# BlockstreamResearch/secp256k1-zkp

Measured on AMD Instinct MI355X. Metric: 64-bit Borromean rangeproof verifies/sec, higher is better.
Workload: dtype u32 limbs (9x29-bit), 32x32->64 integer MAC

## Files before the change

__graft_entry__.py:

```python
import os
import subprocess
import sys

ROOT = os.path.dirname(os.path.abspath(__file__))
CSRC = os.path.join(ROOT, "secp256k1_zkp_amd", "csrc")
HIPCC = os.environ.get("HIPCC", "/opt/rocm/bin/hipcc")
HIP_FLAGS = ["--offload-arch=gfx950", "-O3", "-std=c++17", "-shared", "-fPIC", "-Wno-unused-value"]


def _run(cmd, cwd=None):
    print("+", " ".join(cmd), flush=True)
    subprocess.check_call(cmd, cwd=cwd)


def _stale(target, sources):
    if not os.path.exists(target):
        return True
    t = os.path.getmtime(target)
    return any(os.path.getmtime(s) > t for s in sources if os.path.exists(s))


def build(force=False):
    hdrs = [os.path.join(CSRC, f) for f in os.listdir(CSRC) if f.endswith((".h", ".hip"))] + [os.path.join(ROOT, "include", "secp256k1_zkp_amd.h")]
    sys.path.insert(0, ROOT)
    from secp256k1_zkp_amd import build_lib
    build_lib.build(force=force)
    prims_src = os.path.join(ROOT, "tests", "gpu_prims", "prims.hip")
    prims = os.path.join(ROOT, "tests", "gpu_prims", "libs2k_gpuprims.so")
    if force or _stale(prims, hdrs + [prims_src]):
        _run([HIPCC] + HIP_FLAGS + ["-o", prims, prims_src])
    winv_src = os.path.join(ROOT, "tests", "wave_inverse", "waveinv_test.hip")
    winv = os.path.join(ROOT, "tests", "wave_inverse", "libs2k_waveinv_test.so")
    if force or _stale(winv, hdrs + [winv_src]):
        _run([HIPCC] + HIP_FLAGS + ["-o", winv, winv_src])
    emu_src = os.path.join(ROOT, "tests", "host_emul", "hostemu.cpp")
    emu = os.path.join(ROOT, "tests", "host_emul", "libs2k_hostemu.so")
    if force or _stale(emu, hdrs + [emu_src]):
        _run(["g++", "-O2", "-std=c++17", "-fPIC", "-shared", "-o", emu, emu_src])
    ecdsa_emu_src = os.path.join(ROOT, "tests", "host_emul", "ecdsa_emu.cpp")
    ecdsa_emu = os.path.join(ROOT, "tests", "host_emul", "libs2k_ecdsa_emu.so")
    if force or _stale(ecdsa_emu, hdrs + [emu_src, ecdsa_emu_src]):
        _run(["g++", "-O2", "-std=c++17", "-fPIC", "-shared", "-o", ecdsa_emu, ecdsa_emu_src])
    if os.path.exists(os.path.join(ROOT, "oracle", "zkp_oracle.c")):
        _run(["make", "-s", "-C", os.path.join(ROOT, "oracle"), "oracle"])
    if os.path.isdir(os.environ.get("S2K_REFERENCE", "/root/reference")):
        _run(["make", "-s", "-C", os.path.join(ROOT, "oracle"), "ref", "hooked", "benches", "routed"])
    sys.path.insert(0, ROOT)
    import secp256k1_zkp_amd
    from secp256k1_zkp_amd import _native
    _native.load()


def smoke():
    sys.path.insert(0, ROOT)
    from tests import smoke_impl
    smoke_impl.run()


if __name__ == "__main__":
    build(force="--force" in sys.argv)
    if "--smoke" in sys.argv:
        smoke()
```

secp256k1_zkp_amd/csrc/engine_rangeproof.hip:

```cpp
#include "engine_internal.h"

__global__ void __launch_bounds__(256)
k_rp_header(rp_ws ws, uint64_t* min_value, uint64_t* max_value, const unsigned char* proofs, const uint64_t* proof_off, const unsigned char* gens64,
            rp_gen_dev gc, size_t n) {
    const size_t p = (size_t)blockIdx.x * blockDim.x + threadIdx.x;
    if (p >= n) return;
    if (p == 0) { ws.plan[0] = 0; ws.plan[1] = 0; ws.plan[2] = 0; ws.plan[3] = 0; }
    uint64_t mn, mx;
    rp_header(ws.rec[p], &mn, &mx, proofs + proof_off[p], proof_off[p + 1] - proof_off[p]);
    min_value[p] = mn; max_value[p] = mx;
    ws.rec[p].gslot = rp_gen_lookup(gc, gens64 + 64 * p);
}
__global__ void __launch_bounds__(192)
k_rp_prologue(rp_ws ws, const uint64_t* min_value, const unsigned char* commits33, const unsigned char* proofs,
              const uint64_t* proof_off, const unsigned char* extra, const uint64_t* extra_off, const unsigned char* gens64, size_t n) {
    __builtin_amdgcn_s_setprio(3);
    const u32 role = threadIdx.x >> 6;
    const size_t p = (size_t)blockIdx.x * 64 + (threadIdx.x & 63);
    int commit_ok = 0;
    if (p < n) {
        rp_rec& rec = ws.rec[p];
        if (role == 0) commit_ok = rp_pp_commit(rec, min_value[p], commits33 + 33 * p, gens64 + 64 * p);
        else if (role == 1) {
            const unsigned char* ex = nullptr; uint64_t exlen = 0;
            if (extra && extra_off) { ex = extra + extra_off[p]; exlen = extra_off[p + 1] - extra_off[p]; if (exlen == 0) ex = nullptr; }
            rp_pp_hash(rec, commits33 + 33 * p, proofs + proof_off[p], ex, exlen, gens64 + 64 * p);
        } else rp_pp_bases(rec, ws.bases + p * RP_MAX_RINGS * RP_GEJ_WORDS, gens64 + 64 * p, ws.dbases + p * RP_MAX_RINGS * RP_GEJ_WORDS);
    }
    __syncthreads();
    if (p < n && role == 0 && (ws.rec[p].hdr & 1u) && commit_ok) ws.rec[p].ok = 1;
}
__global__ void __launch_bounds__(256)
k_rp_lift(rp_ws ws, const unsigned char* proofs, const uint64_t* proof_off, size_t n) {
    const size_t t = (size_t)blockIdx.x * blockDim.x + threadIdx.x;
    const size_t p = t >> 5; const u32 ring = (u32)(t & 31);
    if (p >= n) return;
    const rp_rec& rec = ws.rec[p];
    if (!(rec.hdr & 1u) || ring + 1 >= rec.rings) return;
    rp_lift(rec, ws.pub0 + (p * RP_MAX_RINGS + ring) * RP_GEJ_WORDS, ws.lift_ok + p * RP_MAX_RINGS + ring, proofs + proof_off[p], ring);
}
__global__ void __launch_bounds__(64)
k_rp_sum(rp_ws ws, u32 gen_valid, size_t n) {
    const size_t p = (size_t)blockIdx.x * blockDim.x + threadIdx.x;
    u32 cF = 0, cG = 0, rings = 0;
    if (p < n) {
        rp_sum(ws.rec[p], ws.pub0 + p * RP_MAX_RINGS * RP_GEJ_WORDS, ws.lift_ok + p * RP_MAX_RINGS);
        const rp_rec& rec = ws.rec[p];
        if (rec.ok) {
            rings = rec.rings;
            const int fast = gen_valid && rec.gslot < RP_GEN_SLOTS && ((gen_valid >> rec.gslot) & 1u);
            if (fast) cF = (rings + S2K_RP_K - 1) / S2K_RP_K; else cG = rings;
        }
    }
    u32 pf = cF, pg = cG;
    for (int d = 1; d < 64; d <<= 1) {
        const u32 a = __shfl_up(pf, d), b = __shfl_up(pg, d);
        if ((int)threadIdx.x >= d) { pf += a; pg += b; }
    }
    u32 baseF = 0, baseG = 0;
    if (threadIdx.x == 63) { baseF = pf ? atomicAdd(&ws.plan[0], pf) : 0u; baseG = pg ? atomicAdd(&ws.plan[1], pg) : 0u; }
    baseF = __shfl(baseF, 63); baseG = __shfl(baseG, 63);
    u32 oF = baseF + pf - cF, oG = baseG + pg - cG;
    for (u32 g = 0; g < cF; g++) ws.mapF[oF + g] = (u32)p | (g << 20);
    for (u32 r = 0; r < cG; r++) ws.mapG[oG + r] = (u32)p | (r << 20);
}
#ifndef S2K_RINGS_WAVES
#define S2K_RINGS_WAVES 2
#endif
__global__ void __launch_bounds__(256, S2K_RINGS_WAVES)
k_rp_rings_shared(rp_ws ws, const unsigned char* __restrict__ proofs, const uint64_t* __restrict__ proof_off, const u32* __restrict__ gtab, u32* __restrict__ ptab, u32* ev,
                  rp_gen_dev gc, u32 dbg) {
    const size_t t = (size_t)blockIdx.x * blockDim.x + threadIdx.x;
    const u32 nF = ws.plan[0];
    if ((t & ~size_t(63)) >= nF) return;
    const int live = t < nF;
    const u32 item = ws.mapF[live ? t : 0];
    const size_t p = item & 0xFFFFFu; const u32 g = item >> 20;
    const rp_rec& rec = ws.rec[p];
    __shared__ u32 s_dig[S2K_RING_DIG_WORDS * 256];
    const u32 sl = rec.gslot < RP_GEN_SLOTS ? rec.gslot : gc.any;
    const size_t lanes = (size_t)gridDim.x * 256, wave = t >> 6, lane = t & 63;
    u32* const raw0 = ptab + lanes * S2K_RP_K * S2K_RTAB_WORDS;
    const rp_shared_mem M{ptab + t * S2K_RP_K * S2K_RTAB_WORDS, raw0 + wave * S2K_RRAW_WAVE_WORDS + lane,
                          raw0 + (lanes >> 6) * S2K_RRAW_WAVE_WORDS + wave * (S2K_RP_K * RP_PARK_WORDS * 64) + lane, S2K_LANE_DIG(s_dig)};
    const int served = rp_rings_shared<S2K_RP_K>(rec, ws.pub0 + (p * RP_MAX_RINGS + g * S2K_RP_K) * RP_GEJ_WORDS, ws.ring_out + p * RP_RING_OUT_BYTES, ws.ring_ok + p * RP_MAX_RINGS,
                                                 proofs + proof_off[p], g * S2K_RP_K, live, gtab, gc.tab[sl], gc.xmul[sl], M, ev ? ev + p * (RP_MAX_RINGS * 32) : nullptr, dbg);
    if (served != RP_SHARED_SERVED && live) {
        const u32 r0 = g * S2K_RP_K, cnt = rec.rings - r0 < S2K_RP_K ? rec.rings - r0 : S2K_RP_K;
        const u32 base = atomicAdd(&ws.plan[1], cnt);
        for (u32 i = 0; i < cnt; i++) ws.mapG[base + i] = (u32)p | ((r0 + i) << 20);
        atomicAdd(&ws.plan[served == RP_SHARED_SUSPECT ? 2 : 3], cnt);
    }
}
__global__ void __launch_bounds__(256, S2K_RINGS_WAVES)
k_rp_rings(rp_ws ws, const unsigned char* __restrict__ proofs, const uint64_t* __restrict__ proof_off, const u32* __restrict__ gtab, u32* __restrict__ ptab, u32* ev, int split) {
    const size_t t = (size_t)blockIdx.x * blockDim.x + threadIdx.x;
    const u32 nG = ws.plan[1];
    if ((t & ~size_t(63)) >= nG) return;
    const int live = t < nG;
    const u32 item = ws.mapG[live ? t : 0];
    const size_t p = item & 0xFFFFFu; const u32 ring = item >> 20;
    const rp_rec& rec = ws.rec[p];
    __shared__ u32 s_dig[S2K_DIG_WORDS * 256];
    const lane_mem lm{ptab + t * S2K_PTAB_WORDS, S2K_LANE_DIG(s_dig)};
    rp_ring(rec, ws.bases + (p * RP_MAX_RINGS + ring) * RP_GEJ_WORDS, ws.pub0 + (p * RP_MAX_RINGS + ring) * RP_GEJ_WORDS,
            ws.ring_out + p * RP_RING_OUT_BYTES + ring * 33, ws.ring_ok + p * RP_MAX_RINGS + ring, proofs + proof_off[p], ring, live, gtab, lm, ev ? ev + (p * RP_MAX_RINGS + ring) * 32 : nullptr,
            split ? ws.dbases + (p * RP_MAX_RINGS + ring) * RP_GEJ_WORDS : (const u32*)nullptr, split ? ws.tcur + (p * RP_MAX_RINGS + ring) * RP_GEJ_WORDS : (u32*)nullptr);
}
__global__ void __launch_bounds__(64)
k_rp_final(rp_ws ws, int32_t* results, const unsigned char* proofs, const uint64_t* proof_off, const unsigned char* gens64, rp_gen_mbox* mbox, size_t n) {
    const size_t p = (size_t)blockIdx.x * blockDim.x + threadIdx.x;
    int ok = 0; u32 gslot = RP_GSLOT_NONE;
    if (p < n) {
        ok = rp_final(ws.rec[p], ws.ring_out + p * RP_RING_OUT_BYTES, ws.ring_ok + p * RP_MAX_RINGS, proofs + proof_off[p]);
        results[p] = ok;
        gslot = ws.rec[p].gslot;
    }
    if (mbox) {
        for (u32 sl = 0; sl < RP_GEN_SLOTS; sl++) {
            const unsigned long long m = __ballot(ok && gslot == sl);
            if (m && threadIdx.x == 0) atomicAdd(&mbox->hits[sl], (u32)__popcll(m));
        }
        rp_gen_report_miss(mbox, gens64 + 64 * (p < n ? p : 0), ok && gslot == RP_GSLOT_NONE);
    }
}

struct rp_rewind_args {
    u32* ev; u32* prep; u32* secs;
    unsigned char* blind_out; uint64_t* value_out; unsigned char* msg_out; uint64_t* outlen; size_t msg_stride; const unsigned char* nonces;
};
__global__ void __launch_bounds__(64)
k_rp_rewind_draws(rp_ws ws, rp_rewind_args ra, const unsigned char* proofs, const uint64_t* proof_off, const unsigned char* gens64, size_t n) {
    const size_t p = (size_t)blockIdx.x * blockDim.x + threadIdx.x;
    if (p >= n || !ws.rec[p].ok) return;
    rp_rewind_draws(ws.rec[p], proofs + proof_off[p], ra.nonces + 32 * p, gens64 + 64 * p, ra.prep + p * 1024, ra.secs + p * 256);
}
__global__ void __launch_bounds__(256, 2)
k_rp_rewind(rp_ws ws, rp_rewind_args ra, int32_t* results, const uint64_t* min_value, const unsigned char* proofs, const uint64_t* proof_off,
            const unsigned char* gens64, const u32* gtab, u32* ptab, size_t n) {
    const size_t t = (size_t)blockIdx.x * blockDim.x + threadIdx.x;
    const int inrange = t < n;
    const size_t p = inrange ? t : 0;
    int ok = inrange && results[p];
    scalar blind; u64 value = 0, mlen = 0; sc_set_zero(blind);
    const unsigned char* proof = proofs + proof_off[p];
    if (ok) {
        mlen = (ra.msg_out && ra.outlen) ? ra.outlen[p] : 0;
        if (mlen > ra.msg_stride) mlen = ra.msg_stride;
        ok = rp_rewind_recover(blind, value, ra.msg_out ? ra.msg_out + p * ra.msg_stride : nullptr, &mlen, ws.rec[p], proof,
                               ra.ev + p * 1024, ra.prep + p * 1024, ra.secs + p * 256);
    }
    u64 vv = 0;
    if (ok) {
        u32 off; int exp, mant; u64 scale, mn, mx;
        rp_getheader(off, exp, mant, scale, &mn, &mx, proof, proof_off[p + 1] - proof_off[p]);
        vv = value * scale + min_value[p];
    }
    gej A; scalar sv;
    { ge g; fe_set_b32_mod(g.x, gens64 + 64 * p); fe_set_b32_mod(g.y, gens64 + 64 * p + 32); fe_norm_weak(g.x); fe_norm_weak(g.y); gej_set_ge(A, g); }
    sc_set_u64(sv, vv);
    if (!ok) { sc_set_zero(sv); sc_set_zero(blind); }
    __shared__ u32 s_dig[S2K_DIG_WORDS * 256];
    const lane_mem lm{ptab + t * S2K_PTAB_WORDS, S2K_LANE_DIG(s_dig)};
    gej R; ecmult_lane(R, A, sv, blind, 1, gtab, lm);
    ge a; ge_set_gej(a, R);
    if (ok) {
        fe cx, cy, d;
        for (int i = 0; i < 9; i++) { cx.n[i] = ws.rec[p].commit[i]; cy.n[i] = ws.rec[p].commit[9 + i]; }
        ok &= !R.inf;
        fe_neg(d, a.x, 1); fe_add(d, cx); ok &= fe_normalizes_to_zero(d);
        fe_neg(d, a.y, 1); fe_add(d, cy); ok &= fe_normalizes_to_zero(d);
    }
    if (inrange) {
        results[p] = ok;
        if (!ok) { sc_set_zero(blind); vv = 0; mlen = 0; }
        sc_get_b32(ra.blind_out + 32 * p, blind);
        ra.value_out[p] = vv;
        if (ra.outlen) ra.outlen[p] = mlen;
    }
}

static size_t rp_ws_bytes(size_t n) {
    return ws_need({64, (n * RP_MAX_RINGS / S2K_RP_K + 64) * 4, (n * RP_MAX_RINGS + 64) * 4, n * sizeof(rp_rec), n * RP_MAX_RINGS * RP_GEJ_WORDS * 4, n * RP_MAX_RINGS * RP_GEJ_WORDS * 4, n * RP_MAX_RINGS * RP_GEJ_WORDS * 4,
                    n * RP_MAX_RINGS * RP_GEJ_WORDS * 4, n * RP_MAX_RINGS, n * RP_RING_OUT_BYTES, n * RP_MAX_RINGS});
}
static void rp_ws_carve(rp_ws& w, ws_carver& c, size_t n) {
    w.plan = c.take<u32>(16); w.mapF = c.take<u32>(n * RP_MAX_RINGS / S2K_RP_K + 64); w.mapG = c.take<u32>(n * RP_MAX_RINGS + 64);
    w.rec = c.take<rp_rec>(n);
    w.bases = c.take<u32>(n * RP_MAX_RINGS * RP_GEJ_WORDS);
    w.pub0 = c.take<u32>(n * RP_MAX_RINGS * RP_GEJ_WORDS);
    w.dbases = c.take<u32>(n * RP_MAX_RINGS * RP_GEJ_WORDS);
    w.tcur = c.take<u32>(n * RP_MAX_RINGS * RP_GEJ_WORDS);
    w.lift_ok = c.take<unsigned char>(n * RP_MAX_RINGS);
    w.ring_out = c.take<unsigned char>(n * RP_RING_OUT_BYTES);
    w.ring_ok = c.take<unsigned char>(n * RP_MAX_RINGS);
}
int engine_rp_slots(s2k_engine* e, size_t nw) {
    const size_t bytes = (rp_ws_bytes(nw) + (size_t(1) << 20)) & ~((size_t(1) << 20) - 1);
    if (bytes <= e->rp_mem_bytes) return 1;
// ... 504 lines not shown
```

secp256k1_zkp_amd/csrc/group.h:

```cpp
#pragma once
#include "fe.h"

struct ge  { fe x, y; };
struct gej { fe x, y, z; int inf; };

#define GEJ_ADD_NEEDS_DOUBLE 1

S2K_HD void fe_set_beta(fe& r) {
    const u32 b[9] = {0x119501EEu, 0x09CB6143u, 0x1D626570u, 0x0092EA25u, 0x034E99CFu, 0x03CF561Au, 0x1C41B991u, 0x056CAF80u, 0x007AE96Au};
#pragma unroll
    for (int i = 0; i < 9; i++) r.n[i] = b[i];
}

S2K_HD void gej_set_infinity(gej& r) { fe_set_zero(r.x); fe_set_zero(r.y); fe_set_zero(r.z); r.inf = 1; }
S2K_HD void gej_set_ge(gej& r, const ge& a) { r.x = a.x; r.y = a.y; fe_set_int(r.z, 1); r.inf = 0; }
S2K_HD void ge_neg(ge& r, const ge& a) { r.x = a.x; fe_neg(r.y, a.y, 1); fe_norm_weak(r.y); }

S2K_HD void gej_double(gej& r, const gej& a) {
    fe x = a.x, y = a.y, l, s, t;
    fe_norm_weak(x); fe_norm_weak(y);
    fe_mul_sqr(r.z, y, a.z, s, y);
    fe_mul_sqr(t, x, s, l, x);
    fe_neg(t, t, 1);
    fe_mul_int(l, 3); fe_half(l);
    fe_norm_weak(l);
    fe_sqr2(r.x, l, s, s);
    fe_add(r.x, t); fe_add(r.x, t);
    fe_add(t, r.x);
    fe_mul(r.y, t, l);
    fe_add(r.y, s);
    fe_neg(r.y, r.y, 2);
    r.inf = a.inf;
}

S2K_HD int gej_add_ge(gej& r, const gej& a, const ge& b, fe* zr = nullptr) {
    fe z12, u2, s2, h, i, h2, h3, t, i2;
    fe_sqr(z12, a.z);
    fe_mul2(u2, b.x, z12, s2, b.y, z12);
    fe_neg(h, a.x, 5); fe_add(h, u2);
    fe_norm_seq(h);
    fe zz; fe_mul2(s2, s2, a.z, zz, a.z, h);
    fe_neg(i, a.y, 3); fe_add(i, s2);
    fe_norm_seq(i);
    const int hz = fe_seq_is_zero(h), iz = fe_seq_is_zero(i);
    fe_sqr2(i2, i, h2, h);
    fe_mul2(h3, h, h2, t, a.x, h2);
    if (zr) *zr = h;
    fe x3, y3, tn;
    fe_neg(x3, h3, 1);
    fe_neg(tn, t, 1);
    fe_add(x3, tn); fe_add(x3, tn); fe_add(x3, i2);
    fe_norm_weak(x3);
    fe_neg(tn, x3, 1); fe_add(tn, t);
    fe_mul2(y3, tn, i, h3, h3, a.y);
    fe_neg(h3, h3, 1);
    fe_add(y3, h3);
    const int dbl = (!a.inf) & hz & iz;
    const int inf = (!a.inf) & hz & (!iz);
    const int take_b = a.inf | dbl;
    fe one; fe_set_int(one, 1);
    fe_select(r.x, b.x, x3, take_b);
    fe_select(r.y, b.y, y3, take_b);
    fe_select(r.z, one, zz, take_b);
    r.inf = inf;
    return dbl ? GEJ_ADD_NEEDS_DOUBLE : 0;
}

S2K_HD void gej_double_lean(gej& r, const gej& a) {
    fe l, s, t, nx, w;
    fe_mul_sqr(r.z, a.y, a.z, s, a.y);
    fe_neg(nx, a.x, 1);
    fe_mul_sqr(t, nx, s, l, a.x);
    fe_mul_int(l, 3); fe_half(l);
    fe_norm_weak(l);
    fe_sqr(r.x, l);
    fe_add(r.x, t); fe_add(r.x, t);
    fe_norm_weak(r.x);
    fe_add2(w, r.x, t);
    fe_muladd<false, true>(r.y, l, w, s, s);
    fe_neg(r.y, r.y, 1);
    r.inf = 0;
}
S2K_HD int gej_add_ge_lean(gej& r, const gej& a, const ge& b) {
    fe z12, u2, s2, h, i, h2, h3, t, i2, ny, w;
    fe_sqr(z12, a.z);
    fe_mul2(u2, b.x, z12, s2, b.y, z12);
    fe_neg(h, a.x, 1); fe_add(h, u2);
    fe_norm_seq(h);
    fe_mul2(s2, s2, a.z, r.z, a.z, h);
    fe_neg(ny, a.y, 2);
    fe_add2(i, s2, ny);
    fe_norm_weak(i);
    const int hz = fe_seq_is_zero(h);
    fe_sqr2(i2, i, h2, h);
    fe_mul2(h3, h, h2, t, a.x, h2);
    fe_add2(w, t, t); fe_add(w, h3);
    fe_neg(w, w, 3);
    fe_add2(r.x, i2, w);
    fe_norm_weak(r.x);
    fe_neg(w, r.x, 1); fe_add(w, t);
    fe_muladd<false, false>(r.y, i, w, ny, h3);
    r.inf = 0;
    return hz;
}

S2K_HD void gej_add_var(gej& r, const gej& a, const gej& b) {
    fe z22, z12, u1, u2, s1, s2, h, i, h2, h3, t, i2;
    fe_sqr2(z22, b.z, z12, a.z);
    fe_mul2(u1, a.x, z22, u2, b.x, z12);
    fe_mul2(s1, a.y, z22, s2, b.y, z12);
    fe_mul2(s1, s1, b.z, s2, s2, a.z);
    fe_neg(h, u1, 1); fe_add(h, u2);
    fe_neg(i, s1, 1); fe_add(i, s2);
    fe_norm_seq(h); fe_norm_seq(i);
    const int hz = fe_seq_is_zero(h), iz = fe_seq_is_zero(i);
    gej res;
    if ((!a.inf) & (!b.inf) & hz & iz) {
        gej_double(res, a);
    } else {
        fe zz;
        fe_mul_sqr(zz, a.z, b.z, h2, h);
        fe_mul_sqr(res.z, zz, h, i2, i);
        fe_mul2(h3, h, h2, t, u1, h2);
        fe x3, tn;
        fe_neg(x3, h3, 1); fe_neg(tn, t, 1);
        fe_add(x3, tn); fe_add(x3, tn); fe_add(x3, i2);
        fe_norm_weak(x3);
        fe_neg(tn, x3, 1); fe_add(tn, t);
        fe_mul2(res.y, tn, i, h3, h3, s1);
        fe_neg(h3, h3, 1);
        fe_add(res.y, h3);
        res.x = x3;
        res.inf = hz & (!iz);
        if (a.inf) res = b;
        else if (b.inf) res = a;
    }
    r = res;
}

S2K_HD void ge_set_gej(ge& r, const gej& a) {
    fe zi, zi2, zi3;
    fe_inv(zi, a.z);
    fe_sqr(zi2, zi); fe_mul(zi3, zi2, zi);
    fe_mul(r.x, a.x, zi2); fe_mul(r.y, a.y, zi3);
    fe_normalize(r.x); fe_normalize(r.y);
}

S2K_HD void ge_curve_rhs(fe& c, const fe& x) {
    fe x2; fe_sqr(x2, x); fe_mul(c, x2, x);
    c.n[0] += 7u;
}
S2K_HD int ge_set_xquad(ge& r, const fe& x) {
    fe c; ge_curve_rhs(c, x);
    fe_norm_weak(c);
    r.x = x;
    return fe_sqrt(r.y, c);
}
S2K_HD int ge_set_xo(ge& r, const fe& x, int odd) {
    if (!ge_set_xquad(r, x)) return 0;
    fe_normalize(r.y);
    if (fe_is_odd(r.y) != odd) { fe_neg(r.y, r.y, 1); fe_normalize(r.y); }
    return 1;
}
S2K_HD int ge_is_valid(const ge& a) {
    fe y2, c; fe_sqr(y2, a.y); ge_curve_rhs(c, a.x); fe_norm_weak(c);
    return fe_equal(y2, c);
}

struct gez { fe x, y, zz, zzz; int inf; };
S2K_HD void gez_add_ge(gez& a, const ge& b) {
    if (a.inf) { a.x = b.x; a.y = b.y; fe_set_int(a.zz, 1); fe_set_int(a.zzz, 1); a.inf = 0; return; }
    fe u2, s2, p, r;
    fe_mul2(u2, b.x, a.zz, s2, b.y, a.zzz);
    fe_neg(p, a.x, 1); fe_add(p, u2);
    fe_neg(r, a.y, 3); fe_add(r, s2);
    fe_norm_seq(p); fe_norm_seq(r);
    if (fe_seq_is_zero(p)) {
        if (!fe_seq_is_zero(r)) { a.inf = 1; return; }
        gej t, d; gej_set_ge(t, b); gej_double(d, t);
        a.x = d.x; a.y = d.y; fe_norm_weak(a.x); fe_norm_weak(a.y);
        fe_sqr(a.zz, d.z); fe_mul(a.zzz, a.zz, d.z);
        return;
    }
    fe pp, rr, ppp, q;
    fe_sqr2(pp, p, rr, r);
    fe_mul2(ppp, p, pp, q, a.x, pp);
    fe x3, t1, nq, y3a, y3b;
    fe_neg(x3, ppp, 1); fe_neg(nq, q, 1);
    fe_add(x3, nq); fe_add(x3, nq); fe_add(x3, rr);
    fe_norm_weak(x3);
    fe_neg(t1, x3, 1); fe_add(t1, q);
    fe_mul2(y3a, r, t1, y3b, a.y, ppp);
    fe_mul2(a.zz, a.zz, pp, a.zzz, a.zzz, ppp);
    fe_neg(y3b, y3b, 1); fe_add(y3a, y3b);
    a.x = x3; a.y = y3a;
}
S2K_HD void gej_set_gez(gej& r, const gez& a) {
    r.inf = a.inf;
    if (a.inf) { fe_set_zero(r.x); fe_set_zero(r.y); fe_set_zero(r.z); return; }
    fe_mul2(r.x, a.x, a.zz, r.y, a.y, a.zzz);
    r.z = a.zz;
}
S2K_HD void gez_add_ge_lean(gez& a, const ge& b) {
    fe u2, s2, p, r;
    fe_mul2(u2, b.x, a.zz, s2, b.y, a.zzz);
    fe_neg(p, a.x, 1); fe_add(p, u2); fe_norm_weak(p);
    fe_neg(r, a.y, 1); fe_add(r, s2); fe_norm_weak(r);
    fe pp, rr, ppp, q;
    fe_sqr2(pp, p, rr, r);
    fe_mul2(ppp, p, pp, q, a.x, pp);
    fe x3, nq, t1, ny;
    fe_neg(x3, ppp, 1); fe_neg(nq, q, 1);
    fe_add(x3, nq); fe_add(x3, nq); fe_add(x3, rr);
    fe_norm_weak(x3);
    fe_neg(t1, x3, 1); fe_add(t1, q);
    fe_neg(ny, a.y, 1);
    fe_muladd<false, false>(a.y, r, t1, ny, ppp);
    fe_mul2(a.zz, a.zz, pp, a.zzz, a.zzz, ppp);
    a.x = x3;
}
```

secp256k1_zkp_amd/csrc/modinv.h:

```cpp
#pragma once
#include "s2k_common.h"

#define DS_LIMBS 9
#define DS_BITS 30
#define DS_MASK ((int32_t)0x3FFFFFFF)
#define DS_BATCHES 20

struct ds_int { int32_t w[DS_LIMBS]; };
struct ds_modulus { int32_t w[DS_LIMBS]; u32 inv; };

#define DS_MOD_P ds_modulus{{-977, -4, 0, 0, 0, 0, 0, 0, 65536}, 0x2DDACACFu}
#define DS_MOD_N ds_modulus{{0x10364141, 0x3F497A33, 0x348A03BB, 0x2BB739AB, 0x3FFFFEBA, 0x3FFFFFFF, 0x3FFFFFFF, 0x3FFFFFFF, 0xFFFF}, 0x2A774EC1u}

#if defined(__HIP_DEVICE_COMPILE__)
#define DS_WAVE_ANY(p) (__any(p))
#define DS_WAVE_ALL(p) (__all(p))
#define DS_UNIFORM(x) (__builtin_amdgcn_readfirstlane(x))
#else
#define DS_WAVE_ANY(p) (p)
#define DS_WAVE_ALL(p) (p)
#define DS_UNIFORM(x) (x)
#endif

S2K_HD int ds_ctz32(u32 x) { return __builtin_ctz(x | 0x80000000u); }

S2K_HD int32_t ds_batch(int32_t zeta, u32 f, u32 g, int32_t t[4]) {
    int32_t u = 1, v = 0, q = 0, r = 1;
    int left = DS_BITS;
    while (DS_WAVE_ANY(left > 0)) {
        int z = ds_ctz32(g); z = z < left ? z : left;
        g >>= z; u = (int32_t)((u32)u << z); v = (int32_t)((u32)v << z); zeta -= z; left -= z;
        const int act = left > 0;
        const int sw = act & (zeta < 0);
        const u32 fm = sw ? 0u - f : f;
        const int32_t um = sw ? -u : u, vm = sw ? -v : v;
        const u32 g2 = (g + fm) >> 1;
        const int32_t q2 = q + um, r2 = r + vm;
        f = sw ? g : f; u = sw ? q : u; v = sw ? r : v;
        g = act ? g2 : g; q = act ? q2 : q; r = act ? r2 : r;
        zeta = sw ? -zeta - 2 : zeta - act;
        u = (int32_t)((u32)u << act); v = (int32_t)((u32)v << act); left -= act;
    }
    t[0] = u; t[1] = v; t[2] = q; t[3] = r;
    return zeta;
}

S2K_HD int32_t ds_batch_uniform(int32_t zeta, u32 f, u32 g, int32_t t[4]) {
    int32_t u = 1, v = 0, q = 0, r = 1;
    int left = DS_BITS;
    for (;;) {
        int z = ds_ctz32(g); z = z < left ? z : left;
        g >>= z; u = (int32_t)((u32)u << z); v = (int32_t)((u32)v << z); zeta -= z; left -= z;
        if (left <= 0) break;
        if (zeta < 0) {
            const u32 f0 = f; const int32_t u0 = u, v0 = v;
            f = g; u = q; v = r;
            g = (g - f0) >> 1; q -= u0; r -= v0;
            zeta = -zeta - 2;
        } else {
            g = (g + f) >> 1; q += u; r += v;
            zeta -= 1;
        }
        u = (int32_t)((u32)u << 1); v = (int32_t)((u32)v << 1); left -= 1;
    }
    t[0] = u; t[1] = v; t[2] = q; t[3] = r;
    return zeta;
}

template <bool WITH_M>
S2K_HD void ds_apply(ds_int& a, ds_int& b, const int32_t t[4], const ds_modulus md) {
    const int64_t t00 = t[0], t01 = t[1], t10 = t[2], t11 = t[3];
    int64_t ca = t00 * a.w[0] + t01 * b.w[0], cb = t10 * a.w[0] + t11 * b.w[0];
    int64_t ka = 0, kb = 0;
    if (WITH_M) {
        ka = (int64_t)((0u - (u32)ca * md.inv) & (u32)DS_MASK);
        kb = (int64_t)((0u - (u32)cb * md.inv) & (u32)DS_MASK);
        ca += ka * md.w[0]; cb += kb * md.w[0];
    }
    ca >>= DS_BITS; cb >>= DS_BITS;
#pragma unroll
    for (int i = 1; i < DS_LIMBS; i++) {
        ca += t00 * a.w[i] + t01 * b.w[i];
        cb += t10 * a.w[i] + t11 * b.w[i];
        if (WITH_M && md.w[i] != 0) { ca += ka * md.w[i]; cb += kb * md.w[i]; }
        a.w[i - 1] = (int32_t)ca & DS_MASK; ca >>= DS_BITS;
        b.w[i - 1] = (int32_t)cb & DS_MASK; cb >>= DS_BITS;
    }
    a.w[DS_LIMBS - 1] = (int32_t)ca; b.w[DS_LIMBS - 1] = (int32_t)cb;
}

S2K_HD void ds_add_multiple(ds_int& r, int32_t c, const ds_modulus md) {
    int64_t acc = 0;
#pragma unroll
    for (int i = 0; i < DS_LIMBS - 1; i++) { acc += (int64_t)r.w[i] + (int64_t)c * md.w[i]; r.w[i] = (int32_t)acc & DS_MASK; acc >>= DS_BITS; }
    r.w[DS_LIMBS - 1] = (int32_t)(acc + r.w[DS_LIMBS - 1] + (int64_t)c * md.w[DS_LIMBS - 1]);
}

template <bool UNIFORM = false>
S2K_HD void ds_inverse_words(u32 o[8], const u32 w[8], const ds_modulus md) {
    ds_int f, g, d, e;
#pragma unroll
    for (int i = 0; i < DS_LIMBS; i++) {
        const int bit = DS_BITS * i, idx = bit >> 5, sh = bit & 31;
        u64 v = w[idx];
        if (idx + 1 < 8) v |= (u64)w[idx + 1] << 32;
        g.w[i] = (int32_t)((u32)(v >> sh) & (u32)DS_MASK);
        f.w[i] = md.w[i]; d.w[i] = 0; e.w[i] = 0;
    }
    e.w[0] = 1;
    int32_t zeta = -1;
#pragma unroll 1
    for (int it = 0; it < DS_BATCHES; it++) {
        int32_t t[4];
        if (UNIFORM) zeta = ds_batch_uniform(DS_UNIFORM(zeta), (u32)DS_UNIFORM(f.w[0]), (u32)DS_UNIFORM(g.w[0]), t);
        else zeta = ds_batch(zeta, (u32)f.w[0], (u32)g.w[0], t);
        ds_apply<true>(d, e, t, md);
        ds_apply<false>(f, g, t, md);
        if (it >= DS_BATCHES - 5) {
            int32_t gz = 0;
#pragma unroll
            for (int i = 0; i < DS_LIMBS; i++) gz |= g.w[i];
            if (DS_WAVE_ALL(gz == 0)) break;
        }
    }
    ds_add_multiple(d, 32, md);
    const int32_t qest = d.w[DS_LIMBS - 1] >> 16;
    ds_add_multiple(d, -qest, md);
    { ds_int s = d; ds_add_multiple(s, -1, md); const int keep = s.w[DS_LIMBS - 1] >= 0;
#pragma unroll
      for (int i = 0; i < DS_LIMBS; i++) d.w[i] = keep ? s.w[i] : d.w[i]; }
    { const int fneg = f.w[DS_LIMBS - 1] < 0;
      int32_t nz = 0;
#pragma unroll
      for (int i = 0; i < DS_LIMBS; i++) nz |= d.w[i];
      ds_int s;
#pragma unroll
      for (int i = 0; i < DS_LIMBS; i++) s.w[i] = -d.w[i];
      int64_t acc = 0;
#pragma unroll
      for (int i = 0; i < DS_LIMBS - 1; i++) { acc += (int64_t)s.w[i] + md.w[i]; s.w[i] = (int32_t)acc & DS_MASK; acc >>= DS_BITS; }
      s.w[DS_LIMBS - 1] = (int32_t)(acc + s.w[DS_LIMBS - 1] + md.w[DS_LIMBS - 1]);
      const int take = fneg & (nz != 0);
#pragma unroll
      for (int i = 0; i < DS_LIMBS; i++) d.w[i] = take ? s.w[i] : d.w[i]; }
#pragma unroll
    for (int j = 0; j < 8; j++) {
        const int bit = 32 * j, i = bit / DS_BITS, sh = bit % DS_BITS;
        u64 v = (u64)(u32)d.w[i] >> sh;
        if (i + 1 < DS_LIMBS) v |= (u64)(u32)d.w[i + 1] << (DS_BITS - sh);
        if (i + 2 < DS_LIMBS) v |= (u64)(u32)d.w[i + 2] << (2 * DS_BITS - sh);
        o[j] = (u32)v;
    }
}
```

secp256k1_zkp_amd/csrc/rangeproof.h:

```cpp
#pragma once
#include "gtable.h"
#include "sha256.h"
#include "waveinv.h"

#define RP_MAX_RINGS 32
#define RP_GEJ_WORDS 28
#define RP_RING_OUT_BYTES (RP_MAX_RINGS * 33 + 32)
#define RP_GSLOT_NONE 0xFFFFFFFFu

struct rp_rec {
    u32 ok;
    u32 rings;
    u32 last_rsize;
    u32 off_signs;
    u32 off_pts;
    u32 off_e0;
    u32 off_s;
    u32 hdr;
    u32 gslot;
    u32 m[8];
    u32 commit[18];
    u32 accj[RP_GEJ_WORDS];
};

// ... 33 lines not shown
        if (exp > 18) return 0;
        mantissa = proof[offset] + 1;
        if (mantissa > 64) return 0;
        *max_value = 0xFFFFFFFFFFFFFFFFull >> (64 - mantissa);
    } else {
        *max_value = 0;
    }
    offset += 1;
    scale = 1;
    for (int i = 0; i < exp; i++) {
        if (*max_value > 0xFFFFFFFFFFFFFFFFull / 10) return 0;
        *max_value *= 10; scale *= 10;
    }
    *min_value = 0;
    if (has_min) {
        if (plen - offset < 8) return 0;
        u64 v = 0;
        for (int i = 0; i < 8; i++) v = (v << 8) | proof[offset + i];
        *min_value = v;
        offset += 8;
    }
    if (*max_value > 0xFFFFFFFFFFFFFFFFull - *min_value) return 0;
    *max_value += *min_value;
    return 1;
}

S2K_HD void rp_header(rp_rec& rec, u64* min_value, u64* max_value, const unsigned char* proof, u64 plen) {
    rec.ok = 0; rec.rings = 0; rec.last_rsize = 0; rec.hdr = 0; rec.gslot = RP_GSLOT_NONE;
    rec.off_signs = 0; rec.off_pts = 0; rec.off_e0 = 0; rec.off_s = 0;
    *min_value = 0; *max_value = 0;
    u32 offset; int exp, mantissa; u64 scale;
    if (!rp_getheader(offset, exp, mantissa, scale, min_value, max_value, proof, plen)) return;
    u32 rings = 1, npub = 1, last_rsize = 1;
    if (mantissa != 0) {
        rings = (u32)mantissa >> 1; npub = rings * 4; last_rsize = 4;
        if (mantissa & 1) { npub += 2; rings++; last_rsize = 2; }
    }
    if (plen - offset < (u64)32 * (npub + rings - 1) + 32 + ((rings + 6) >> 3)) return;
    rec.rings = rings; rec.last_rsize = last_rsize;
    rec.off_signs = offset;
    offset += (rings + 6) >> 3;
    if ((rings - 1) & 7) {
        if ((proof[offset - 1] >> ((rings - 1) & 7)) != 0) return;
    }
    rec.off_pts = offset;
    rec.off_e0 = offset + 32 * (rings - 1);
    rec.off_s = rec.off_e0 + 32;
    if ((u64)rec.off_s + (u64)32 * npub != plen) return;
    rec.hdr = 1u | ((u32)(exp + 1) << 8);
}
S2K_HD void rp_load_generator(ge& g, const unsigned char* gen64) {
    fe_set_b32_mod(g.x, gen64); fe_set_b32_mod(g.y, gen64 + 32);
    fe_normalize(g.x); fe_normalize(g.y);
}
S2K_HD int rp_pp_commit(rp_rec& rec, u64 min_value, const unsigned char* commit33, const unsigned char* gen64) {
    if (!(rec.hdr & 1u)) return 0;
    ge c;
    int valid = (commit33[0] & 0xFEu) == 8u;
    {
        fe x; valid &= fe_set_b32_limit(x, commit33 + 1);
        valid &= ge_set_xquad(c, x);
        fe_normalize(c.x); fe_normalize(c.y);
        if (commit33[0] & 1) { fe_neg(c.y, c.y, 1); fe_normalize(c.y); }
    }
    for (int i = 0; i < 9; i++) { rec.commit[i] = c.x.n[i]; rec.commit[9 + i] = c.y.n[i]; }
    gej acc; gej_set_infinity(acc);
    if (min_value) {
        ge g; rp_load_generator(g, gen64);
        for (int bit = 63; bit >= 0; bit--) {
            gej t; gej_double(t, acc); acc = t;
            if ((min_value >> bit) & 1) {
                const int f = gej_add_ge(t, acc, g); acc = t;
                if (f == GEJ_ADD_NEEDS_DOUBLE) { gej_double(t, acc); acc = t; }
            }
        }
    }
    gej_store28_h(rec.accj, acc);
    return valid;
}
S2K_HD void rp_pp_hash(rp_rec& rec, const unsigned char* commit33, const unsigned char* proof, const unsigned char* extra, u64 extra_len,
                       const unsigned char* gen64) {
    if (!(rec.hdr & 1u)) return;
    const u32 rings = rec.rings, off_hdr = rec.off_signs;
    ge g; rp_load_generator(g, gen64);
    sha256_stream h; sha256_stream_init(h);
    unsigned char buf[32];
    fe cx; fe_set_b32_mod(cx, commit33 + 1); fe_normalize(cx);
    fe rhs; ge_curve_rhs(rhs, cx);
    const int cy_zero = fe_normalizes_to_zero(rhs);
    sha256_stream_put(h, (unsigned char)((commit33[0] & 1) && !cy_zero ? 1 : 0));
    fe_get_b32(buf, cx); sha256_stream_write(h, buf, 32);
    fe r; const int gsq = fe_sqrt(r, g.y);
    sha256_stream_put(h, (unsigned char)(!gsq));
    fe_get_b32(buf, g.x); sha256_stream_write(h, buf, 32);
    sha256_stream_write(h, proof, off_hdr);
    for (u32 i = 0; i + 1 < rings; i++) {
        const unsigned char sign = (proof[rec.off_signs + (i >> 3)] & (1u << (i & 7))) != 0;
        sha256_stream_put(h, sign);
        sha256_stream_write(h, proof + rec.off_pts + 32 * i, 32);
    }
    if (extra) sha256_stream_write(h, extra, (size_t)extra_len);
    unsigned char m[32];
    sha256_stream_finalize(h, m);
    for (int i = 0; i < 8; i++) rec.m[i] = s2k_load_be32(m + 4 * i);
}
S2K_HD void rp_pp_bases(const rp_rec& rec, u32* bases , const unsigned char* gen64, u32* dbases = nullptr ) {
    if (!(rec.hdr & 1u)) return;
    const u32 rings = rec.rings;
    const int exp = (int)((rec.hdr >> 8) & 0xFFu) - 1;
    ge g; rp_load_generator(g, gen64);
    gej base; ge ng; ng.x = g.x; fe_neg(ng.y, g.y, 1); fe_norm_weak(ng.y);
    gej_set_ge(base, ng);
    for (int e = 0; e < exp; e++) {
        gej t2, t8, s;
        gej_double(t2, base); gej_double(t8, t2); gej_double(s, t8);
        gej_add_var(base, s, t2);
    }
    fe_norm_weak(base.x); fe_norm_weak(base.y);
    const u32 total = dbases ? rings + 32 : rings;
    for (u32 i = 0; i < total; i++) {
        if (i < rings) gej_store28_h(bases + RP_GEJ_WORDS * i, base);
        if (dbases && i >= 32) gej_store28_h(dbases + RP_GEJ_WORDS * (i - 32), base);
        if (i + 1 < total) { gej_double_lean(base, base); gej_double_lean(base, base); }
    }
}
S2K_HD void rp_prologue_points(rp_rec& rec, u32* bases , u64 min_value, const unsigned char* commit33,
                               const unsigned char* proof, const unsigned char* extra, u64 extra_len, const unsigned char* gen64, u32* dbases = nullptr) {
    if (!(rec.hdr & 1u)) return;
    const int commit_ok = rp_pp_commit(rec, min_value, commit33, gen64);
    rp_pp_hash(rec, commit33, proof, extra, extra_len, gen64);
    rp_pp_bases(rec, bases, gen64, dbases);
    rec.ok = (u32)commit_ok;
}

S2K_HD void rp_prologue(rp_rec& rec, u32* bases, u64* min_value, u64* max_value, const unsigned char* commit33,
                        const unsigned char* proof, u64 plen, const unsigned char* extra, u64 extra_len, const unsigned char* gen64, u32* dbases = nullptr) {
    rp_header(rec, min_value, max_value, proof, plen);
    rp_prologue_points(rec, bases, *min_value, commit33, proof, extra, extra_len, gen64, dbases);
}

S2K_HD void rp_lift(const rp_rec& rec, u32* pub0_ring, unsigned char* lift_ok, const unsigned char* proof, u32 ring) {
    fe x; ge c;
    const unsigned char* px = proof + rec.off_pts + 32 * ring;
    int ok = fe_set_b32_limit(x, px);
    ok &= ge_set_xquad(c, x);
    const int sign = (proof[rec.off_signs + (ring >> 3)] >> (ring & 7)) & 1;
    fe ny; fe_neg(ny, c.y, 1);
    fe_select(c.y, ny, c.y, sign);
    gej j; gej_set_ge(j, c);
    gej_store28_h(pub0_ring, j);
    *lift_ok = (unsigned char)ok;
}

S2K_HD void rp_sum(rp_rec& rec, u32* pub0 , const unsigned char* lift_ok ) {
    if (!rec.ok) return;
    gej acc; gej_load28_h(acc, rec.accj);
    int ok = 1;
    for (u32 i = 0; i + 1 < rec.rings; i++) {
        ok &= lift_ok[i];
        gej c; gej_load28_h(c, pub0 + RP_GEJ_WORDS * i);
        ge ca; ca.x = c.x; ca.y = c.y;
        gej t; const int f = gej_add_ge(t, acc, ca); acc = t;
        if (f == GEJ_ADD_NEEDS_DOUBLE) { gej_double(t, acc); acc = t; }
    }
    fe ny; fe_neg(ny, acc.y, 3); fe_norm_weak(ny); acc.y = ny;
    fe_norm_weak(acc.x);
    ge cm;
    for (int i = 0; i < 9; i++) { cm.x.n[i] = rec.commit[i]; cm.y.n[i] = rec.commit[9 + i]; }
    gej last; const int f = gej_add_ge(last, acc, cm);
    if (f == GEJ_ADD_NEEDS_DOUBLE) { gej t; gej_double(t, last); last = t; }
    if (last.inf) ok = 0;
    else { ge a; ge_set_gej(a, last); gej_set_ge(last, a); }
    gej_store28_h(pub0 + RP_GEJ_WORDS * (rec.rings - 1), last);
    if (!ok) rec.ok = 0;
}

S2K_HD void rp_words_to_scalar(scalar& s, int& overflow, const u32 w[8]) {
#pragma unroll
    for (int i = 0; i < 8; i++) s.d[i] = w[7 - i];
    overflow = sc_check_overflow(s.d);
    sc_reduce_once(s.d, overflow);
}
S2K_HD void rp_hash_e0(u32 out[8], const u32 e0[8], const u32 m[8], u32 ring) {
    u32 st[8], w[16];
    sha256_init(st);
#pragma unroll
    for (int i = 0; i < 8; i++) { w[i] = e0[i]; w[8 + i] = m[i]; }
    sha256_compress(st, w);
    w[0] = ring; w[1] = 0; w[2] = 0x80000000u;
#pragma unroll
    for (int i = 3; i < 15; i++) w[i] = 0;
    w[15] = 72 * 8;
    sha256_compress(st, w);
#pragma unroll
    for (int i = 0; i < 8; i++) out[i] = st[i];
}
S2K_HD void rp_hash_step(u32 out[8], u32 prefix, const u32 x[8], const u32 m[8], u32 ring, u32 epos) {
    u32 st[8], w[16];
    sha256_init(st);
    w[0] = (prefix << 24) | (x[0] >> 8);
#pragma unroll
    for (int i = 1; i < 8; i++) w[i] = (x[i - 1] << 24) | (x[i] >> 8);
    w[8] = (x[7] << 24) | (m[0] >> 8);
#pragma unroll
    for (int i = 1; i < 8; i++) w[8 + i] = (m[i - 1] << 24) | (m[i] >> 8);
    sha256_compress(st, w);
    w[0] = (m[7] << 24) | (ring >> 8);
    w[1] = (ring << 24) | (epos >> 8);
    w[2] = (epos << 24) | 0x00800000u;
#pragma unroll
    for (int i = 3; i < 15; i++) w[i] = 0;
    w[15] = 73 * 8;
    sha256_compress(st, w);
#pragma unroll
    for (int i = 0; i < 8; i++) out[i] = st[i];
}

S2K_HD void rp_ring(const rp_rec& rec, const u32* base28, u32* pub28, unsigned char* ring_out33, unsigned char* ring_ok,
                    const unsigned char* proof, u32 ring, int live, const u32* gtab, const lane_mem& lm, u32* ev_out = nullptr,
                    const u32* dbase28 = nullptr, u32* t28 = nullptr) {
    const u32 rsize = (ring + 1 == rec.rings) ? rec.last_rsize : 4u;
    int ok = live & (int)rec.ok;
    u32 e[8];
    {
        u32 m[8];
#pragma unroll
        for (int i = 0; i < 8; i++) m[i] = rec.m[i];
        u32 e0[8] = {0, 0, 0, 0, 0, 0, 0, 0};
        if (ok) {
            const unsigned char* pe0 = proof + rec.off_e0;
#pragma unroll
            for (int i = 0; i < 8; i++) e0[i] = s2k_load_be32(pe0 + 4 * i);
        }
        rp_hash_e0(e, e0, m, ring);
    }
    u32 outx[8] = {0, 0, 0, 0, 0, 0, 0, 0}; u32 outp = 0;
    S2K_PROF_DECL;
    if (t28) {
        gej t; gej_load28_h(t, pub28);
        const int tinf = t.inf; t.inf = 0;
#pragma unroll 1
        for (int k = 0; k < 64; k++) gej_double_lean(t, t);
        fe_norm_weak(t.y);
        t.inf = tinf;
        if (live) gej_store28_h(t28, t);
    }
    S2K_PROF_MARK(11);
#pragma unroll 1
    for (u32 j = 0; j < 4; j++) {
        const int step_live = ok & (j < rsize);
        scalar ens, s; int ov_e, ov_s = 0;
        if (ev_out && live) { for (int i = 0; i < 8; i++) ev_out[8 * j + i] = e[i]; }
        rp_words_to_scalar(ens, ov_e, e);
        sc_set_zero(s);
        if (step_live) sc_set_b32(s, proof + rec.off_s + 32 * (4 * ring + j), &ov_s);
        gej pub; gej_load28_h(pub, pub28);
        int good = step_live & !ov_e & !ov_s & !sc_is_zero(s) & !sc_is_zero(ens) & !pub.inf;
        if (!good) { sc_set_zero(ens); sc_set_zero(s); }
        gej T; if (t28) gej_load28_h(T, t28);
        if (j + 1 < rsize) {
            gej base, nxt; gej_load28_h(base, base28);
            gej_add_var(nxt, pub, base);
            if (live) gej_store28_h(pub28, nxt);
            if (t28) { gej_load28_h(base, dbase28); gej_add_var(nxt, T, base); if (live) gej_store28_h(t28, nxt); }
        }
        gej R;
        S2K_PROF_MARK(0);
        int split_done = 0;
        if (t28) split_done = ecmult_lane_split(R, pub, T, ens, s, 1, gtab, lm);
        if (!S2K_WAVE_ALL(split_done)) ecmult_lane(R, pub, ens, s, 1, gtab, lm);
        S2K_PROF_RESET;
        good &= !R.inf;
        ge a; ge_set_gej(a, R);
        S2K_PROF_MARK(4);
        u32 xw[8]; fe_to_words(xw, a.x);
        u32 xb[8];
#pragma unroll
        for (int i = 0; i < 8; i++) xb[i] = xw[7 - i];
        const u32 prefix = 2u | (u32)fe_is_odd(a.y);
        if (step_live) ok &= good;
        if (j + 1 < rsize) {
            u32 m[8];
#pragma unroll
            for (int i = 0; i < 8; i++) m[i] = rec.m[i];
            rp_hash_step(e, prefix, xb, m, ring, j + 1);
        } else if (j + 1 == rsize) {
#pragma unroll
            for (int i = 0; i < 8; i++) outx[i] = xb[i];
            outp = prefix;
        }
        S2K_PROF_MARK(5);
    }
    if (live) {
        ring_out33[0] = (unsigned char)outp;
        for (int i = 0; i < 8; i++) s2k_store_be32(ring_out33 + 1 + 4 * i, outx[i]);
        *ring_ok = (unsigned char)ok;
    }
}

#define RP_GEN_SLOTS 8
#define RP_GEN_MBOX 4
struct rp_gen_dev {
    const u32* tab[RP_GEN_SLOTS];
    const u32* xmul[RP_GEN_SLOTS];
    const unsigned char* keys;
    u32 valid;
    u32 any;
};
struct rp_gen_mbox { unsigned long long tag[RP_GEN_MBOX]; u32 count[RP_GEN_MBOX]; u32 hits[RP_GEN_SLOTS]; unsigned char key[RP_GEN_MBOX][64]; };
S2K_HD unsigned long long rp_gen_tag(const unsigned char* gen64) {
    unsigned long long h = 0xCBF29CE484222325ull;
    for (int k = 0; k < 64; k++) { h ^= gen64[k]; h *= 0x100000001B3ull; }
    return h ? h : 1ull;
}
S2K_HD u32 rp_gen_lookup(const rp_gen_dev& gc, const unsigned char* gen64) {
    u32 slot = RP_GSLOT_NONE;
    for (u32 i = 0; i < RP_GEN_SLOTS; i++) {
        if (!((gc.valid >> i) & 1u)) continue;
        int same = 1;
        for (int k = 0; k < 64; k++) same &= (gc.keys[64 * i + k] == gen64[k]);
        if (same) slot = i;
    }
    return slot;
}
#if defined(__HIPCC__) || defined(__HIP__)
__device__ __forceinline__ void rp_gen_report_miss(rp_gen_mbox* mb, const unsigned char* gen64, int report) {
    const unsigned long long mask = __ballot(report);
// ... 234 lines not shown
```

secp256k1_zkp_amd/csrc/waveinv.h:

```cpp
#pragma once
#include "fe.h"

#if defined(__HIPCC__)
S2K_D u32 wi_lane() { return (u32)(threadIdx.x & 63u); }
S2K_D void wi_fetch(fe& r, const fe& a, u32 src) {
    const int addr = (int)(src << 2);
#pragma unroll
    for (int i = 0; i < FE_LIMBS; i++) r.n[i] = (u32)__builtin_amdgcn_ds_bpermute(addr, (int)a.n[i]);
}
S2K_D int fe_inv_wave(fe& r, const fe& z) {
    const u32 l = wi_lane();
    fe pre = z, suf = z;
#pragma unroll
    for (int s = 0; s < 6; s++) {
        const u32 d = 1u << s;
        fe a, b, pa, sb;
        wi_fetch(a, pre, (l - d) & 63u);
        wi_fetch(b, suf, (l + d) & 63u);
        fe_mul2(pa, pre, a, sb, suf, b);
        fe_cmov(pre, pa, l >= d);
        fe_cmov(suf, sb, l + d < 64u);
    }
    fe e, s, one, q, P;
    fe_set_int(one, 1);
    wi_fetch(e, pre, (l - 1u) & 63u); fe_cmov(e, one, l == 0u);
    wi_fetch(s, suf, (l + 1u) & 63u); fe_cmov(s, one, l == 63u);
    fe_mul(q, e, s);
    wi_fetch(P, pre, 63u);
    fe_normalize(P);
    const int ok = !fe_is_zero_normalized(P);
    u32 w[8], o[8]; fe_to_words(w, P);
    ds_inverse_words<true>(o, w, DS_MOD_P);
    fe ip; fe_from_words(ip, o);
    fe_mul(r, ip, q);
    return ok;
}
#endif

S2K_HD int fe_inv_lanes(fe& r, const fe& z) {
#if defined(__HIP_DEVICE_COMPILE__)
    return fe_inv_wave(r, z);
#else
    fe_inv(r, z);
    return !fe_normalizes_to_zero(z);
#endif
}
```

Before: 1.080 million.

## Batch rangeproof sum affine conversion via wave inverse with lane-distributed divsteps

k_rp_sum now splits rp_sum into a key phase and a store phase so that each lane's z-coordinate inversion goes through the wavefront-batched inverse (prefix/suffix products plus one shared inversion), replacing a per-thread fe_inv. The shared inversion itself now runs in a new lane-distributed safegcd variant by default. That variant spreads the limb updates across lanes using DPP carries and readlane broadcasts instead of having every lane do the full scalar limb arithmetic. The cost is cross-lane shuffles and extra multiplications, plus a fallback fe_inv when the wave product is zero. Inactive lanes feed z=1 into the batch.

Result: faster. 1.092 million (median of 6 runs) (+1.2%).

```diff
diff --git a/__graft_entry__.py b/__graft_entry__.py
--- a/__graft_entry__.py
+++ b/__graft_entry__.py
@@ -33,6 +33,10 @@
     winv = os.path.join(ROOT, "tests", "wave_inverse", "libs2k_waveinv_test.so")
     if force or _stale(winv, hdrs + [winv_src]):
         _run([HIPCC] + HIP_FLAGS + ["-o", winv, winv_src])
+    wlanes_src = os.path.join(ROOT, "tests", "wave_inverse", "waveinv_lanes_test.hip")
+    wlanes = os.path.join(ROOT, "tests", "wave_inverse", "libs2k_waveinv_lanes_test.so")
+    if force or _stale(wlanes, hdrs + [wlanes_src]):
+        _run([HIPCC] + HIP_FLAGS + ["-o", wlanes, wlanes_src])
     emu_src = os.path.join(ROOT, "tests", "host_emul", "hostemu.cpp")
     emu = os.path.join(ROOT, "tests", "host_emul", "libs2k_hostemu.so")
     if force or _stale(emu, hdrs + [emu_src]):
diff --git a/secp256k1_zkp_amd/csrc/engine_rangeproof.hip b/secp256k1_zkp_amd/csrc/engine_rangeproof.hip
--- a/secp256k1_zkp_amd/csrc/engine_rangeproof.hip
+++ b/secp256k1_zkp_amd/csrc/engine_rangeproof.hip
@@ -43,8 +43,17 @@
 k_rp_sum(rp_ws ws, u32 gen_valid, size_t n) {
     const size_t p = (size_t)blockIdx.x * blockDim.x + threadIdx.x;
     u32 cF = 0, cG = 0, rings = 0;
+    const int active = p < n && ws.rec[p < n ? p : 0].ok;
+    gej last; int sum_ok = 1, finite = 0;
+    fe z; fe_set_int(z, 1);
+    if (active) {
+        finite = rp_sum_key(last, sum_ok, ws.rec[p], ws.pub0 + p * RP_MAX_RINGS * RP_GEJ_WORDS, ws.lift_ok + p * RP_MAX_RINGS);
+        if (finite) z = last.z;
+    }
+    fe zi;
+    if (!fe_inv_lanes(zi, z)) fe_inv(zi, z);
+    if (active) rp_sum_store(ws.rec[p], ws.pub0 + p * RP_MAX_RINGS * RP_GEJ_WORDS, last, sum_ok, zi);
     if (p < n) {
-        rp_sum(ws.rec[p], ws.pub0 + p * RP_MAX_RINGS * RP_GEJ_WORDS, ws.lift_ok + p * RP_MAX_RINGS);
         const rp_rec& rec = ws.rec[p];
         if (rec.ok) {
             rings = rec.rings;
diff --git a/secp256k1_zkp_amd/csrc/group.h b/secp256k1_zkp_amd/csrc/group.h
--- a/secp256k1_zkp_amd/csrc/group.h
+++ b/secp256k1_zkp_amd/csrc/group.h
@@ -138,12 +138,16 @@
     r = res;
 }
 
-S2K_HD void ge_set_gej(ge& r, const gej& a) {
-    fe zi, zi2, zi3;
-    fe_inv(zi, a.z);
+S2K_HD void ge_set_gej_zinv(ge& r, const gej& a, const fe& zi) {
+    fe zi2, zi3;
     fe_sqr(zi2, zi); fe_mul(zi3, zi2, zi);
     fe_mul(r.x, a.x, zi2); fe_mul(r.y, a.y, zi3);
     fe_normalize(r.x); fe_normalize(r.y);
+}
+S2K_HD void ge_set_gej(ge& r, const gej& a) {
+    fe zi;
+    fe_inv(zi, a.z);
+    ge_set_gej_zinv(r, a, zi);
 }
 
 S2K_HD void ge_curve_rhs(fe& c, const fe& x) {
diff --git a/secp256k1_zkp_amd/csrc/modinv.h b/secp256k1_zkp_amd/csrc/modinv.h
--- a/secp256k1_zkp_amd/csrc/modinv.h
+++ b/secp256k1_zkp_amd/csrc/modinv.h
@@ -96,6 +96,37 @@
     r.w[DS_LIMBS - 1] = (int32_t)(acc + r.w[DS_LIMBS - 1] + (int64_t)c * md.w[DS_LIMBS - 1]);
 }
 
+S2K_HD void ds_finish_words(u32 o[8], const ds_int& f, ds_int& d, const ds_modulus md) {
+    ds_add_multiple(d, 32, md);
+    const int32_t qest = d.w[DS_LIMBS - 1] >> 16;
+    ds_add_multiple(d, -qest, md);
+    { ds_int s = d; ds_add_multiple(s, -1, md); const int keep = s.w[DS_LIMBS - 1] >= 0;
+#pragma unroll
+      for (int i = 0; i < DS_LIMBS; i++) d.w[i] = keep ? s.w[i] : d.w[i]; }
+    { const int fneg = f.w[DS_LIMBS - 1] < 0;
+      int32_t nz = 0;
+#pragma unroll
+      for (int i = 0; i < DS_LIMBS; i++) nz |= d.w[i];
+      ds_int s;
+#pragma unroll
+      for (int i = 0; i < DS_LIMBS; i++) s.w[i] = -d.w[i];
+      int64_t acc = 0;
+#pragma unroll
+      for (int i = 0; i < DS_LIMBS - 1; i++) { acc += (int64_t)s.w[i] + md.w[i]; s.w[i] = (int32_t)acc & DS_MASK; acc >>= DS_BITS; }
+      s.w[DS_LIMBS - 1] = (int32_t)(acc + s.w[DS_LIMBS - 1] + md.w[DS_LIMBS - 1]);
+      const int take = fneg & (nz != 0);
+#pragma unroll
+      for (int i = 0; i < DS_LIMBS; i++) d.w[i] = take ? s.w[i] : d.w[i]; }
+#pragma unroll
+    for (int j = 0; j < 8; j++) {
+        const int bit = 32 * j, i = bit / DS_BITS, sh = bit % DS_BITS;
+        u64 v = (u64)(u32)d.w[i] >> sh;
+        if (i + 1 < DS_LIMBS) v |= (u64)(u32)d.w[i + 1] << (DS_BITS - sh);
+        if (i + 2 < DS_LIMBS) v |= (u64)(u32)d.w[i + 2] << (2 * DS_BITS - sh);
+        o[j] = (u32)v;
+    }
+}
+
 template <bool UNIFORM = false>
 S2K_HD void ds_inverse_words(u32 o[8], const u32 w[8], const ds_modulus md) {
     ds_int f, g, d, e;
@@ -123,32 +154,67 @@
             if (DS_WAVE_ALL(gz == 0)) break;
         }
     }
-    ds_add_multiple(d, 32, md);
-    const int32_t qest = d.w[DS_LIMBS - 1] >> 16;
-    ds_add_multiple(d, -qest, md);
-    { ds_int s = d; ds_add_multiple(s, -1, md); const int keep = s.w[DS_LIMBS - 1] >= 0;
-#pragma unroll
-      for (int i = 0; i < DS_LIMBS; i++) d.w[i] = keep ? s.w[i] : d.w[i]; }
-    { const int fneg = f.w[DS_LIMBS - 1] < 0;
-      int32_t nz = 0;
-#pragma unroll
-      for (int i = 0; i < DS_LIMBS; i++) nz |= d.w[i];
-      ds_int s;
-#pragma unroll
-      for (int i = 0; i < DS_LIMBS; i++) s.w[i] = -d.w[i];
-      int64_t acc = 0;
-#pragma unroll
-      for (int i = 0; i < DS_LIMBS - 1; i++) { acc += (int64_t)s.w[i] + md.w[i]; s.w[i] = (int32_t)acc & DS_MASK; acc >>= DS_BITS; }
-      s.w[DS_LIMBS - 1] = (int32_t)(acc + s.w[DS_LIMBS - 1] + md.w[DS_LIMBS - 1]);
-      const int take = fneg & (nz != 0);
-#pragma unroll
-      for (int i = 0; i < DS_LIMBS; i++) d.w[i] = take ? s.w[i] : d.w[i]; }
-#pragma unroll
-    for (int j = 0; j < 8; j++) {
-        const int bit = 32 * j, i = bit / DS_BITS, sh = bit % DS_BITS;
-        u64 v = (u64)(u32)d.w[i] >> sh;
-        if (i + 1 < DS_LIMBS) v |= (u64)(u32)d.w[i + 1] << (DS_BITS - sh);
-        if (i + 2 < DS_LIMBS) v |= (u64)(u32)d.w[i + 2] << (2 * DS_BITS - sh);
-        o[j] = (u32)v;
-    }
-}
+    ds_finish_words(o, f, d, md);
+}
+
+#if defined(__HIPCC__)
+S2K_D int32_t dsl_from_below(int32_t x) { return __builtin_amdgcn_update_dpp(0, x, 0x111, 0xf, 0xf, true); }
+S2K_D int32_t dsl_from_above(int32_t x) { return __builtin_amdgcn_update_dpp(0, x, 0x101, 0xf, 0xf, true); }
+S2K_D int32_t dsl_carry(int64_t s, int32_t lm, int32_t cm) {
+    const int32_t lo = (int32_t)s & DS_MASK, mid = (int32_t)(s >> DS_BITS) & lm, top = (int32_t)(s >> (2 * DS_BITS));
+    const int32_t u = dsl_from_above(lo) + mid;
+    const int32_t c = ((u >> DS_BITS) + top) & cm;
+    return (u & lm) + dsl_from_below(c);
+}
+S2K_D void dsl_gather(ds_int& r, int32_t v) {
+#pragma unroll
+    for (int i = 0; i < DS_LIMBS; i++) r.w[i] = __builtin_amdgcn_readlane(v, i);
+}
+
+template <bool DUMP = false>
+S2K_D void ds_inverse_words_lanes(u32 o[8], const u32 w[8], const ds_modulus md, int32_t* dump = nullptr, int* batches = nullptr) {
+    const u32 lane = (u32)(threadIdx.x & 63u);
+    const int32_t lm = lane < DS_LIMBS - 1 ? DS_MASK : -1, cm = lane < DS_LIMBS - 1 ? -1 : 0;
+    int32_t m = 0, f, g = 0, d = 0, e = lane == 0 ? 1 : 0;
+#pragma unroll
+    for (int i = 0; i < DS_LIMBS; i++) {
+        const int bit = DS_BITS * i, idx = bit >> 5, sh = bit & 31;
+        u64 v = w[idx];
+        if (idx + 1 < 8) v |= (u64)w[idx + 1] << 32;
+        g = lane == (u32)i ? (int32_t)((u32)(v >> sh) & (u32)DS_MASK) : g;
+        if (md.w[i] != 0) m = lane == (u32)i ? md.w[i] : m;
+    }
+    f = m;
+    int32_t zeta = -1;
+    int it = 0;
+#pragma unroll 1
+    for (; it < DS_BATCHES; it++) {
+        int32_t t[4];
+        zeta = ds_batch_uniform(DS_UNIFORM(zeta), (u32)__builtin_amdgcn_readlane(f, 0), (u32)__builtin_amdgcn_readlane(g, 0), t);
+        const u32 d0 = (u32)__builtin_amdgcn_readlane(d, 0), e0 = (u32)__builtin_amdgcn_readlane(e, 0);
+        const int32_t ka = (int32_t)((0u - ((u32)t[0] * d0 + (u32)t[1] * e0) * md.inv) & (u32)DS_MASK);
+        const int32_t kb = (int32_t)((0u - ((u32)t[2] * d0 + (u32)t[3] * e0) * md.inv) & (u32)DS_MASK);
+        const int64_t sd = (int64_t)t[0] * d + (int64_t)t[1] * e + (int64_t)ka * m, se = (int64_t)t[2] * d + (int64_t)t[3] * e + (int64_t)kb * m;
+        const int64_t sf = (int64_t)t[0] * f + (int64_t)t[1] * g, sg = (int64_t)t[2] * f + (int64_t)t[3] * g;
+        d = dsl_carry(sd, lm, cm); e = dsl_carry(se, lm, cm);
+        f = dsl_carry(sf, lm, cm); g = dsl_carry(sg, lm, cm);
+        if (DUMP) {
+            if (lane < DS_LIMBS) {
+                int32_t* p = dump + (size_t)4 * DS_LIMBS * it + lane;
+                p[0] = f; p[DS_LIMBS] = g; p[2 * DS_LIMBS] = d; p[3 * DS_LIMBS] = e;
+            }
+        }
+        if (it >= DS_BATCHES - 5) {
+            int32_t z = g;
+#pragma unroll
+            for (int k = 0; k < DS_LIMBS - 1; k++) z = (z & lm) + dsl_from_below((z >> DS_BITS) & cm);
+            if (__all(z == 0)) { it++; break; }
+        }
+    }
+    if (DUMP) *batches = it;
+    ds_int fw, dw;
+    dsl_gather(fw, f); dsl_gather(dw, d);
+    ds_add_multiple(fw, 0, md);
+    ds_finish_words(o, fw, dw, md);
+}
+#endif
diff --git a/secp256k1_zkp_amd/csrc/rangeproof.h b/secp256k1_zkp_amd/csrc/rangeproof.h
--- a/secp256k1_zkp_amd/csrc/rangeproof.h
+++ b/secp256k1_zkp_amd/csrc/rangeproof.h
@@ -209,10 +209,9 @@
     *lift_ok = (unsigned char)ok;
 }
 
-S2K_HD void rp_sum(rp_rec& rec, u32* pub0 , const unsigned char* lift_ok ) {
-    if (!rec.ok) return;
+S2K_HD int rp_sum_key(gej& last, int& ok, const rp_rec& rec, const u32* pub0 , const unsigned char* lift_ok ) {
     gej acc; gej_load28_h(acc, rec.accj);
-    int ok = 1;
+    ok = 1;
     for (u32 i = 0; i + 1 < rec.rings; i++) {
         ok &= lift_ok[i];
         gej c; gej_load28_h(c, pub0 + RP_GEJ_WORDS * i);
@@ -224,12 +223,22 @@
     fe_norm_weak(acc.x);
     ge cm;
     for (int i = 0; i < 9; i++) { cm.x.n[i] = rec.commit[i]; cm.y.n[i] = rec.commit[9 + i]; }
-    gej last; const int f = gej_add_ge(last, acc, cm);
+    const int f = gej_add_ge(last, acc, cm);
     if (f == GEJ_ADD_NEEDS_DOUBLE) { gej t; gej_double(t, last); last = t; }
     if (last.inf) ok = 0;
-    else { ge a; ge_set_gej(a, last); gej_set_ge(last, a); }
+    return !last.inf;
+}
+S2K_HD void rp_sum_store(rp_rec& rec, u32* pub0, gej& last, int ok, const fe& zi) {
+    if (!last.inf) { ge a; ge_set_gej_zinv(a, last, zi); gej_set_ge(last, a); }
     gej_store28_h(pub0 + RP_GEJ_WORDS * (rec.rings - 1), last);
     if (!ok) rec.ok = 0;
+}
+S2K_HD void rp_sum(rp_rec& rec, u32* pub0 , const unsigned char* lift_ok ) {
+    if (!rec.ok) return;
+    gej last; int ok;
+    fe zi; fe_set_zero(zi);
+    if (rp_sum_key(last, ok, rec, pub0, lift_ok)) fe_inv(zi, last.z);
+    rp_sum_store(rec, pub0, last, ok, zi);
 }
 
 S2K_HD void rp_words_to_scalar(scalar& s, int& overflow, const u32 w[8]) {
diff --git a/secp256k1_zkp_amd/csrc/waveinv.h b/secp256k1_zkp_amd/csrc/waveinv.h
--- a/secp256k1_zkp_amd/csrc/waveinv.h
+++ b/secp256k1_zkp_amd/csrc/waveinv.h
@@ -8,6 +8,12 @@
 #pragma unroll
     for (int i = 0; i < FE_LIMBS; i++) r.n[i] = (u32)__builtin_amdgcn_ds_bpermute(addr, (int)a.n[i]);
 }
+#if defined(S2K_WAVEINV_SCALAR_APPLY)
+#define WI_SCALAR_APPLY true
+#else
+#define WI_SCALAR_APPLY false
+#endif
+template <bool SCALAR_APPLY = WI_SCALAR_APPLY>
 S2K_D int fe_inv_wave(fe& r, const fe& z) {
     const u32 l = wi_lane();
     fe pre = z, suf = z;
@@ -30,7 +36,8 @@
     fe_normalize(P);
     const int ok = !fe_is_zero_normalized(P);
     u32 w[8], o[8]; fe_to_words(w, P);
-    ds_inverse_words<true>(o, w, DS_MOD_P);
+    if (SCALAR_APPLY) ds_inverse_words<true>(o, w, DS_MOD_P);
+    else ds_inverse_words_lanes(o, w, DS_MOD_P);
     fe ip; fe_from_words(ip, o);
     fe_mul(r, ip, q);
     return ok;
```
